# sideprotocol/plonky2-gpu

Measured on AMD Instinct MI355X. Metric: NTTs/sec at 2^20 Goldilocks, higher is better.
Workload: dtype u64 (Goldilocks, integer modular)

## Files before the change

plonky2_gpu_amd/csrc/capi.hip:

```cpp
#include <algorithm>
#include <list>
#include <map>
#include <mutex>
#include <string>
#include <vector>

#include <stdio.h>
#include <stdlib.h>
#include <string.h>

#include "../../include/plonky2_hip.h"
#include "gl_field.h"
#include "knobs.h"
#include "keccak.h"
#include "merkle.h"
#include "ntt.h"
#include "ntt_kernels.h"
#include "plonk.h"
#include "stark.h"
#include "fri.h"
#include "ed25519_gate_program.inc"

using namespace plonky2_hip;

// ... 1166 lines not shown

GlError gl_merkle_tree_from_columns_h(uint32_t hasher, const uint64_t *d_cols, uint32_t leaf_len, uint64_t n_leaves, uint64_t col_stride,
                                      uint32_t cap_height, uint64_t *d_digests, uint64_t *d_cap, void *ctx) {
    if (hasher == GL_HASHER_POSEIDON) return gl_merkle_tree_from_columns(d_cols, leaf_len, n_leaves, col_stride, cap_height, d_digests, d_cap, ctx);
    if (hasher != GL_HASHER_KECCAK25) return fail(GL_E_INVALID, "unknown hasher");
    DeviceCall device_call(ctx);
    if (!ctx || (!d_cols && leaf_len) || !d_cap) return fail(GL_E_INVALID, "null pointer");
    if (n_leaves == 0 || (n_leaves & (n_leaves - 1))) return fail(GL_E_INVALID, "n_leaves must be a power of two");
    if (cap_height > 63 || (1ull << cap_height) > n_leaves) return fail(GL_E_INVALID, "cap_height should be at most log2(leaves.len())");
    if ((1ull << cap_height) < n_leaves && !d_digests) return fail(GL_E_INVALID, "null pointer");
    if (leaf_len > 1 && col_stride < n_leaves) return fail(GL_E_INVALID, "col_stride smaller than n_leaves: the columns would overlap");
    if (leaf_len == 4) return fail(GL_E_INVALID, KECCAK_LEAF_LEN_4);
    HIP_TRY(keccak_merkle_tree(d_cols, 1, col_stride, leaf_len, n_leaves, cap_height, d_digests, d_cap, S(ctx)->stream));
    return ok();
}

GlError gl_merkle_tree_from_leaves_h(uint32_t hasher, const uint64_t *d_rows, uint32_t leaf_len, uint64_t n_leaves, uint32_t cap_height,
                                     uint64_t *d_digests, uint64_t *d_cap, void *ctx) {
    if (hasher == GL_HASHER_POSEIDON) return gl_merkle_tree_from_leaves(d_rows, leaf_len, n_leaves, cap_height, d_digests, d_cap, ctx);
    if (hasher != GL_HASHER_KECCAK25) return fail(GL_E_INVALID, "unknown hasher");
    DeviceCall device_call(ctx);
    if (!ctx || (!d_rows && leaf_len) || !d_cap) return fail(GL_E_INVALID, "null pointer");
    if (n_leaves == 0 || (n_leaves & (n_leaves - 1))) return fail(GL_E_INVALID, "n_leaves must be a power of two");
    if (cap_height > 63 || (1ull << cap_height) > n_leaves) return fail(GL_E_INVALID, "cap_height should be at most log2(leaves.len())");
    if ((1ull << cap_height) < n_leaves && !d_digests) return fail(GL_E_INVALID, "null pointer");
    if (leaf_len == 4) return fail(GL_E_INVALID, KECCAK_LEAF_LEN_4);
    HIP_TRY(keccak_merkle_tree(d_rows, leaf_len, 1, leaf_len, n_leaves, cap_height, d_digests, d_cap, S(ctx)->stream));
    return ok();
}

GlError gl_commit_from_coeffs_h(uint32_t hasher, const uint64_t *d_coeffs, uint64_t poly_num, uint32_t log_n, uint32_t rate_bits,
                                uint32_t cap_height, uint32_t salt_size, uint64_t shift, uint64_t *d_lde, uint64_t *d_leaves,
                                uint64_t *d_digests, uint64_t *d_cap, void *ctx) {
    if (hasher == GL_HASHER_POSEIDON)
        return gl_commit_from_coeffs(d_coeffs, poly_num, log_n, rate_bits, cap_height, salt_size, shift, d_lde, d_leaves, d_digests, d_cap, ctx);
    if (hasher != GL_HASHER_KECCAK25) return fail(GL_E_INVALID, "unknown hasher");
    DeviceCall device_call(ctx);
    return commit_from_coeffs_keccak(d_coeffs, poly_num, log_n, rate_bits, cap_height, salt_size, shift, d_lde, d_leaves, d_digests, d_cap, S(ctx));
}

GlError gl_commit_from_values_h(uint32_t hasher, uint64_t *d_values, uint64_t poly_num, uint32_t log_n, uint32_t rate_bits,
                                uint32_t cap_height, uint32_t salt_size, uint64_t shift, uint64_t *d_lde, uint64_t *d_leaves,
                                uint64_t *d_digests, uint64_t *d_cap, void *ctx) {
    if (hasher == GL_HASHER_POSEIDON)
        return gl_commit_from_values(d_values, poly_num, log_n, rate_bits, cap_height, salt_size, shift, d_lde, d_leaves, d_digests, d_cap, ctx);
    if (hasher != GL_HASHER_KECCAK25) return fail(GL_E_INVALID, "unknown hasher");
    DeviceCall device_call(ctx);
    if (const char *why = keccak_commit_argument_error(d_values, poly_num, log_n, rate_bits, cap_height, salt_size, d_lde, d_digests, d_cap, ctx))
        return fail(GL_E_INVALID, why);
    GlError e = gl_ntt_batch(d_values, poly_num, log_n, 1ull << log_n, 1, 0, ctx);
    if (e.code) return e;
    return gl_commit_from_coeffs_h(hasher, d_values, poly_num, log_n, rate_bits, cap_height, salt_size, shift, d_lde, d_leaves, d_digests, d_cap, ctx);
}

GlError gl_debug_copy(void *d_dst, const void *d_src, uint64_t bytes, void *ctx) {
    DeviceCall device_call(ctx);
    if (!ctx || !d_dst || !d_src) return fail(GL_E_INVALID, "null pointer");
    if ((bytes & 15) || (((uintptr_t)d_dst | (uintptr_t)d_src) & 15)) return fail(GL_E_INVALID, "16-byte granularity");
    if (bytes == 0) return ok();
    const uint64_t n16 = bytes / 16, per_block = 256ull * COPY_UNROLL;
    hipLaunchKernelGGL(copy16_kernel, dim3((unsigned)((n16 + per_block - 1) / per_block)), dim3(256), 0, S(ctx)->stream,
                       static_cast<const uint64_t *>(d_src), static_cast<uint64_t *>(d_dst), n16);
    HIP_TRY(hipGetLastError());
    return ok();
}

__global__ void radix_probe_kernel(int which, const uint64_t *in, uint64_t *out, uint64_t n_vec) {
    const uint64_t i = (uint64_t)blockIdx.x * blockDim.x + threadIdx.x;
    const uint64_t j = i < n_vec ? i : n_vec - 1;
    uint64_t v[16];
#pragma unroll
    for (int k = 0; k < 16; k++) v[k] = in[j * 16 + k];
    using namespace nttk;
    switch (which) {
        case 0: radix_dif_stage<4, 0, 0>(v); break;
        case 1: radix_dif_stage<4, 0, 1>(v); break;
        case 2: radix_dif_stage<4, 0, 2>(v); break;
        case 3: radix_dif_stage<4, 0, 3>(v); break;
        case 4: radix_dif<4, 0>(v); break;
        case 5: radix_dif_blocks<2>(v); break;
        case 6: shift_twiddles_radix4<0>(v); break;
        case 7: shift_twiddles_radix4<1>(v); break;
        case 8: shift_twiddles_radix4<2>(v); break;
        default: shift_twiddles_radix4<3>(v); break;
    }
    if (i < n_vec)
#pragma unroll
        for (int k = 0; k < 16; k++) out[i * 16 + k] = gl::canon(v[k]);
}

GlError gl_debug_field_op(int op, const uint64_t *d_a, const uint64_t *d_b, uint64_t *d_out, uint64_t n, void *ctx) {
    DeviceCall device_call(ctx);
    if (!ctx || !d_a || !d_out) return fail(GL_E_INVALID, "null pointer");
    if (n == 0) return ok();
    if (op >= 100 && op < 110) {
        if (n % 16) return fail(GL_E_INVALID, "ops 100-109 take vectors of sixteen elements");
        const uint64_t n_vec = n / 16;
        hipLaunchKernelGGL(radix_probe_kernel, dim3((unsigned)((n_vec + 255) / 256)), dim3(256), 0, S(ctx)->stream, op - 100, d_a, d_out, n_vec);
        HIP_TRY(hipGetLastError());
        return ok();
    }
    hipLaunchKernelGGL(field_op_kernel, dim3((unsigned)((n + 255) / 256)), dim3(256), 0, S(ctx)->stream, op, d_a, d_b,
                       d_out, n);
    HIP_TRY(hipGetLastError());
    return ok();
}


void init(void) {
    if (hipSetDevice(0) != hipSuccess) return;
    std::lock_guard<std::mutex> lk(g_mu);
    const NttTables *tb;
    (void)device_tables(0, &tb);
}

GlError ifft(uint64_t *d_values_flatten, int poly_num, int values_num_per_poly, int log_len,
             const uint64_t *d_root_table, const uint64_t *n_inv, void *ctx) {
    DeviceCall device_call(ctx);
    (void)d_root_table;
    if (poly_num < 0 || log_len < 0 || values_num_per_poly != (1 << log_len)) return fail(GL_E_INVALID, "bad sizes");
    if (n_inv) {
        uint64_t expect = glh::P - ((glh::P - 1) >> log_len);
        if (*n_inv % glh::P != expect) return fail(GL_E_INVALID, "n_inv does not equal 2^-log_len");
    }
    GlError e = gl_ntt_batch(d_values_flatten, (uint64_t)poly_num, (uint32_t)log_len, (uint64_t)values_num_per_poly, 1, 0, ctx);
    if (e.code) return e;
    HIP_TRY(hipStreamSynchronize(S(ctx)->stream));
    return ok();
}

GlError merkle_tree_from_coeffs(uint64_t *d_values_flatten, uint64_t *d_ext_values_flatten, int poly_num,
                                int values_num_per_poly, int log_len, const uint64_t *d_root_table,
                                const uint64_t *d_root_table2, const uint64_t *d_shift_powers, int rate_bits,
                                int salt_size, int cap_height, int pad_extvalues_len, void *ctx) {
    DeviceCall device_call(ctx);
    (void)d_root_table;
    (void)d_root_table2;
    (void)d_shift_powers;
    if (poly_num <= 0 || log_len < 0 || rate_bits < 0 || salt_size < 0 || cap_height < 0 || pad_extvalues_len < 0 ||
        values_num_per_poly != (1 << log_len))
        return fail(GL_E_INVALID, "bad sizes");
    if (log_len > 24) return fail(GL_E_INVALID, "log_len > 24 is not supported by this build");
    const uint64_t n_ext = (uint64_t)values_num_per_poly << rate_bits;
    const uint64_t ext_polys = (uint64_t)poly_num + salt_size;
    if ((uint64_t)pad_extvalues_len < ext_polys * n_ext)
        return fail(GL_E_INVALID, "pad_extvalues_len smaller than (poly_num+salt_size)*n_ext: regions would overlap");
    uint64_t *region_b = d_ext_values_flatten + pad_extvalues_len;
    uint64_t *digests = region_b + ext_polys * n_ext;
    uint64_t num_digests = 2 * (n_ext - (1ull << cap_height));
    GlError e = commit_from_coeffs_impl(d_values_flatten, (uint64_t)poly_num, (uint32_t)log_len, (uint32_t)rate_bits,
                                        (uint32_t)cap_height, (uint32_t)salt_size, 7, region_b, d_ext_values_flatten,
                                        digests, digests + 4 * num_digests, S(ctx), true);
    if (e.code) return e;
    HIP_TRY(hipStreamSynchronize(S(ctx)->stream));
    if (!PLONKY2_KNOB("PLONKY2_DROP_STREAM2_WAIT")) HIP_TRY(hipStreamSynchronize(S(ctx)->stream2));
    return ok();
}

GlError merkle_tree_from_values(uint64_t *d_values_flatten, uint64_t *d_ext_values_flatten, int poly_num,
                                int values_num_per_poly, int log_len, const uint64_t *d_root_table,
                                const uint64_t *d_root_table2, const uint64_t *d_shift_powers, const uint64_t *n_inv,
                                int rate_bits, int salt_size, int cap_height, int pad_extvalues_len, void *ctx) {
    DeviceCall device_call(ctx);
    GlError e = ifft(d_values_flatten, poly_num, values_num_per_poly, log_len, d_root_table, n_inv, ctx);
    if (e.code) return e;
    return merkle_tree_from_coeffs(d_values_flatten, d_ext_values_flatten, poly_num, values_num_per_poly, log_len,
                                   d_root_table, d_root_table2, d_shift_powers, rate_bits, salt_size, cap_height,
                                   pad_extvalues_len, ctx);
}

GlError build_merkle_tree(uint64_t *d_ext_values_flatten, int poly_num, int values_num_per_poly, int log_len,
                          int rate_bits, int salt_size, int cap_height, int pad_extvalues_len, void *ctx) {
    DeviceCall device_call(ctx);
    if (!ctx || !d_ext_values_flatten) return fail(GL_E_INVALID, "null pointer");
    if (poly_num <= 0 || log_len < 0 || rate_bits < 0 || salt_size < 0 || cap_height < 0 || pad_extvalues_len < 0 ||
        values_num_per_poly != (1 << log_len) || cap_height > log_len + rate_bits)
        return fail(GL_E_INVALID, "bad sizes");
    const uint32_t log_ext = (uint32_t)(log_len + rate_bits);
    const uint64_t n_ext = 1ull << log_ext, ext_polys = (uint64_t)poly_num + salt_size;
// ... 169 lines not shown
```

plonky2_gpu_amd/csrc/ntt_direct.hip:

```cpp

#include "ntt_kernels.h"

namespace plonky2_hip {
namespace nttk {

namespace {

#ifndef NTT_TAIL_GROUPED
#define NTT_TAIL_GROUPED 1
#endif
#ifndef DIRECT_DIAG_HOOKS
#define DIRECT_TILE_BARRIER() lds_barrier()
#define DIRECT_LOAD_TILE(t) (t)
#define DIRECT_STORE_TILE(t) (t)
#define DIRECT_DIAG_TAIL_FRONT_ON 0
#define DIRECT_DIAG_SAME_STORES_ON 0
#define DIRECT_NT_LOAD_COL false
#define DIRECT_NT_STORE_COL false
#define DIRECT_NT_LOAD_ROW false
#define DIRECT_NT_STORE_ROW false
#define DIRECT_TOUCH_STATE
#define DIRECT_TOUCH_COL(t_in_a)
#define DIRECT_TOUCH_ROW(t_in_a)
#endif

__device__ __forceinline__ uint64_t lds_ld(const unsigned char *lds, uint32_t off) { return *reinterpret_cast<const uint64_t *>(lds + off); }
__device__ __forceinline__ void lds_st(unsigned char *lds, uint32_t off, uint64_t v) { *reinterpret_cast<uint64_t *>(lds + off) = v; }
template <bool NT = false>
__device__ __forceinline__ uint64_t g_ld(const uint64_t *base, uint32_t byte_off) {
    const uint64_t *q = reinterpret_cast<const uint64_t *>(reinterpret_cast<const unsigned char *>(base) + byte_off);
    if constexpr (NT) return __builtin_nontemporal_load(q);
    return *q;
}
template <bool NT = false>
__device__ __forceinline__ void g_st(uint64_t *base, uint32_t byte_off, uint64_t v) {
    uint64_t *q = reinterpret_cast<uint64_t *>(reinterpret_cast<unsigned char *>(base) + byte_off);
    if constexpr (NT)
        __builtin_nontemporal_store(v, q);
    else
        *q = v;
}
constexpr bool NT_LOAD_COL = DIRECT_NT_LOAD_COL, NT_STORE_COL = DIRECT_NT_STORE_COL, NT_LOAD_ROW = DIRECT_NT_LOAD_ROW, NT_STORE_ROW = DIRECT_NT_STORE_ROW;

template <int LOGG>
struct ColGeom {
    static constexpr int G = 1 << LOGG, LOGC = 6 - LOGG, C = 1 << LOGC, LOGR = 8 + LOGG, R = 1 << LOGR;
    static constexpr uint32_t ROWB = C * 8;
    static constexpr uint32_t SA = 16 * ROWB + (G >= 4 ? ROWB : 0);
    static constexpr uint32_t XBYTES = 16 * G * SA;
    static constexpr uint32_t TWBYTES = 16 * G * 16 * 8;
    static constexpr uint32_t LDS_BYTES = XBYTES + TWBYTES;
    static constexpr uint32_t cu_entries(uint32_t gz) { return gz * (G > 1 ? G * 16 : 256); }
    static constexpr uint32_t t2z_entries(uint32_t gz) { return G > 1 ? gz * 16 * G : 0; }
    static constexpr uint32_t cs_entries(uint32_t gz) { return gz * C; }
    static constexpr uint32_t coset_bytes(uint32_t gz) { return (cu_entries(gz) + t2z_entries(gz) + cs_entries(gz)) * 8; }
};

static_assert(ColGeom<3>::LDS_BYTES <= 160 * 1024 && ColGeom<2>::LDS_BYTES <= 160 * 1024, "the exchange image and the tables must fit the 160 KiB of LDS of a gfx950 CU");

template <int LOGG, bool NATURAL, bool COSET = false, bool FINAL = false, bool REVIN = false>
__global__ __launch_bounds__(1024) __attribute__((amdgpu_waves_per_eu(4, 4))) void ntt_col_direct_kernel(const PassParams p, const uint32_t gx, const uint32_t gy, const uint32_t gz, const uint32_t per_b) {
    using GEO = ColGeom<LOGG>;
    constexpr int G = GEO::G, LOGC = GEO::LOGC, C = GEO::C, LOGR = GEO::LOGR;
    constexpr uint32_t ROWB = GEO::ROWB, SA = GEO::SA;
    extern __shared__ __attribute__((aligned(16))) unsigned char ldsb[];
    unsigned char *X = ldsb;
    unsigned char *TW = ldsb + GEO::XBYTES;
    unsigned char *CU = TW + GEO::TWBYTES, *T2Z = CU + GEO::cu_entries(gz) * 8, *CS = T2Z + GEO::t2z_entries(gz) * 8;

    const uint32_t tid = threadIdx.x, lane = tid & 63;
    const uint32_t wave = __builtin_amdgcn_readfirstlane(tid >> 6);
    const uint32_t g = lane >> LOGC, c = lane & (C - 1);

    const uint32_t W = gridDim.x;
    const uint32_t u = (W & 7) == 0 ? (blockIdx.x & 7) * (W >> 3) + (blockIdx.x >> 3) : blockIdx.x;
    const uint32_t P = gy * gz;
    uint32_t b0, bstep, p0, pstep;
    if (per_b) {
        if constexpr (COSET) b0 = u / per_b, p0 = u % per_b;
        else b0 = u % gx, p0 = u / gx;
        bstep = gx, pstep = per_b;
    } else {
        b0 = u, bstep = W, p0 = 0, pstep = 1;
    }
    const uint32_t np_local = p0 < P ? (P - p0 + pstep - 1) / pstep : 0;
    const uint32_t nb_local = b0 < gx ? (gx - b0 + bstep - 1) / bstep : 0;
    const uint32_t n_tiles = np_local * nb_local;
    if (n_tiles == 0) return;

    for (uint32_t e = tid; e < 16u * G * 16u; e += 1024) {
        const uint32_t w_ = e / (16 * G), g_ = (e / 16) % G, ka = e % 16;
        reinterpret_cast<uint64_t *>(TW)[e] = p.twh[(ka * (16 * g_ + w_)) << (12 - LOGR)];
    }
    uint64_t t2[G > 1 ? G : 1];
    if constexpr (!COSET)
        static_for<1, G>([&](auto K_) {
            constexpr int kb = decltype(K_)::value;
            t2[kb] = p.twh[(kb * wave) << (12 - 4 - LOGG)];
        });
    if constexpr (COSET) {
        auto cs_pow = [&](uint32_t z, uint64_t ex) { return gl::mul(p.cs_hi[z * p.cs_hi_len + (uint32_t)(ex >> 10)], p.cs_lo[z * 1024 + (uint32_t)(ex & 1023)]); };
        for (uint32_t e = tid; e < GEO::cu_entries(gz); e += 1024) {
            const uint32_t i = e & 15, mid = G > 1 ? 16 * ((e >> 4) % G) : (e >> 4) & 15, z = G > 1 ? e / (16 * G) : e >> 8;
            reinterpret_cast<uint64_t *>(CU)[e] = cs_pow(z, (uint64_t)p.in_m * (((uint32_t)i << (LOGR - 4)) + mid));
        }
        for (uint32_t e = tid; e < GEO::t2z_entries(gz); e += 1024) {
            const uint32_t kb = e % G, w_ = (e / G) & 15, z = e / (16 * G);
            reinterpret_cast<uint64_t *>(T2Z)[e] = gl::mul(p.twh[(kb * w_) << (12 - 4 - LOGG)], cs_pow(z, (uint64_t)p.in_m * w_));
        }
        for (uint32_t e = tid; e < GEO::cs_entries(gz); e += 1024)
            reinterpret_cast<uint64_t *>(CS)[e] = cs_pow(e / C, (uint64_t)b0 * C + (e % C));
    }

    const uint32_t tw_base = (wave * G + g) * 128;
    const uint32_t lane_x = wave * ROWB + c * 8;
    const uint32_t pw_base = 16 * g * SA + lane_x;
    const uint32_t pr_base = g * SA + lane_x;
    constexpr bool natural = NATURAL;
    auto opaque_lane = [&]() {
        uint32_t l = lane;
        asm volatile("" : "+v"(l));
        return l;
    };
    auto kab_of = [&](uint32_t l) { return G * wave + (l >> LOGC); };
    auto xr_base_of = [&](uint32_t l) { return kab_of(l) * SA + (l & (C - 1)) * 8; };
    auto ld_off_of = [&](uint32_t l) { return (uint32_t)(((l & (C - 1)) + (uint64_t)(16 * (l >> LOGC) + wave) * p.in_m) * 8); };
    const uint64_t out_c = p.out_c ? p.out_c : 1;
    auto st_off_of = [&](uint32_t l) {
        const uint32_t kab = kab_of(l);
        const uint32_t out_row_lane = natural ? kab : (brev_rt(kab & 15, 4) << (LOGR - 4)) | (brev_rt(kab >> 4, LOGG) << 4);
        return (uint32_t)(((l & (C - 1)) * out_c + (uint64_t)out_row_lane * p.out_m) * 8);
    };

    auto tile_of = [&](uint32_t t, uint32_t &b, uint32_t &a, uint32_t &z) {
        const uint32_t bi = t / np_local, pi = t - bi * np_local;
        b = b0 + bi * bstep;
        const uint32_t pp = p0 + pi * pstep;
        if constexpr (COSET) a = pp / gz, z = pp % gz;
        else a = pp % gy, z = pp / gy;
        if (p.sweep_down) a = gy - 1 - a;
    };

    uint64_t A[16];
    const uint32_t ld_step = (uint32_t)(((uint64_t)p.in_m << (LOGR - 4)) * 8);
    auto issue_loads = [&](uint32_t t) {
        uint32_t b, a, z;
        tile_of(DIRECT_LOAD_TILE(t), b, a, z);
        if constexpr (REVIN) {
            static_assert(!COSET && NATURAL, "the reversed-input pass is the first pass of a natural-order inverse transform");
            const uint64_t *base = p.src + (a * p.in_sa + z * p.in_sz);
            const uint32_t l = opaque_lane();
            const uint32_t L = b * C + (l & (C - 1)), m0 = 16 * (l >> LOGC) + wave;
            const uint32_t cols = (uint32_t)p.in_m;
            uint32_t off = L ? (((uint32_t)GEO::R - 1 - m0) * cols + (cols - L)) * 8 : (((uint32_t)GEO::R - m0) * cols) * 8;
            const bool wraps = L == 0 && m0 == 0;
            static_for<0, 16>([&](auto I_) {
                constexpr int i = decltype(I_)::value;
                if constexpr (i == 0) A[i] = g_ld<NT_LOAD_COL>(base, wraps ? 0u : off);
                else A[i] = g_ld<NT_LOAD_COL>(base, off);
                if constexpr (i < 15) off -= ld_step;
            });
            return;
        }
        const uint64_t *base = p.src + (a * p.in_sa + b * p.in_sb + z * p.in_sz);
        uint32_t off = ld_off_of(opaque_lane());
        static_for<0, 16>([&](auto I_) {
            constexpr int i = decltype(I_)::value;
            A[i] = g_ld<NT_LOAD_COL>(base, off);
            if constexpr (i < 15) off += ld_step;
        });
    };

    uint64_t B[16];
    uint64_t cc0 = 1, cstep = 1;
    constexpr bool kept_twiddles = !COSET && !FINAL;
    uint64_t cw[kept_twiddles ? 8 : 1], cstep8 = 1;
    uint32_t chain_b = 0xFFFFFFFFu;
    const uint32_t st_row = (uint32_t)(p.out_m * 8);

    uint64_t cc = 1;
    uint64_t *obase = p.dst;
    uint32_t so = 0;
    auto tail_begin = [&](uint32_t k) {
        uint32_t b, a, z;
        tile_of(k, b, a, z);
        if (!FINAL && b != chain_b) {
            chain_b = b;
            const uint32_t l = opaque_lane();
            const uint64_t L = (uint64_t)b * C + (l & (C - 1));
            cc0 = wpow(p, L * kab_of(l));
            if (p.chain_scale != 1) cc0 = gl::mul(cc0, p.chain_scale);
            cstep = wpow(p, L << (4 + LOGG));
            asm volatile("" : "+v"(cc0), "+v"(cstep));
            if constexpr (kept_twiddles) {
                cw[0] = cc0;
                static_for<1, 8>([&](auto J_) {
                    constexpr int j = decltype(J_)::value;
                    cw[j] = gl::mul(cw[j - 1], cstep);
                });
                const uint64_t s2 = gl::mul(cstep, cstep), s4 = gl::mul(s2, s2);
                cstep8 = gl::mul(s4, s4);
            }
        }
        if constexpr (DIRECT_DIAG_SAME_STORES_ON) tile_of(0, b, a, z);
        obase = p.dst + (a * p.out_sa + b * p.out_sb + (COSET ? brev_rt(z, p.rate_bits) : z) * p.out_sz);
        if constexpr (COSET) cc = gl::mul(cc0, lds_ld(CS, (z * C + (opaque_lane() & (C - 1))) * 8));
        else cc = cc0;
        so = st_off_of(opaque_lane());
    };
    auto tail_unit = [&](auto J_) {
        constexpr int j = decltype(J_)::value;
        constexpr int s3 = brev_c(j, 4);
        if constexpr (FINAL) {
            B[s3] = gl::canon(B[s3]);
        } else if constexpr (kept_twiddles) {
            if constexpr (j < 8) B[s3] = gl::mul(B[s3], cw[j]);
            else B[s3] = gl::mul(B[s3], gl::mul(cw[j - 8], cstep8));
        } else {
            B[s3] = gl::mul(B[s3], cc);
            if constexpr (j < 15) cc = gl::mul(cc, cstep);
        }
        const uint32_t row = natural ? (uint32_t)(j << (4 + LOGG)) : (uint32_t)s3;
        g_st<NT_STORE_COL>(obase, so + row * st_row, B[s3]);
        __builtin_amdgcn_sched_barrier(0);
    };
    auto tail_store = [&](auto J_) {
        constexpr int j = decltype(J_)::value;
        constexpr int s3 = brev_c(j, 4);
        const uint32_t row = natural ? (uint32_t)(j << (4 + LOGG)) : (uint32_t)s3;
        g_st<NT_STORE_COL>(obase, so + row * st_row, B[s3]);
        __builtin_amdgcn_sched_barrier(0);
    };
    auto tail_units = [&](auto LO_, auto HI_) {
        constexpr int LO = decltype(LO_)::value, HI = decltype(HI_)::value, N = HI - LO;
        if constexpr (NTT_TAIL_GROUPED && kept_twiddles && N >= 1 && N <= 8) {
            uint64_t tw[N];
            constexpr int N_HI = HI > 8 ? HI - (LO > 8 ? LO : 8) : 0;
            if constexpr (N_HI > 0)
                rare_group<N_HI>([&](auto I_, gl::rare_mask &f) { constexpr int j = (LO > 8 ? LO : 8) + decltype(I_)::value; tw[j - LO] = gl::mul_f(cw[j - 8], cstep8, f); },
                                 [&](auto I_, gl::rare_mask f) { constexpr int j = (LO > 8 ? LO : 8) + decltype(I_)::value; tw[j - LO] = gl::mul_fix(tw[j - LO], f); });
            rare_group<N>(
                [&](auto I_, gl::rare_mask &f) {
                    constexpr int j = LO + decltype(I_)::value, s3 = brev_c(j, 4);
                    if constexpr (j < 8) B[s3] = gl::mul_f(B[s3], cw[j], f);
                    else B[s3] = gl::mul_f(B[s3], tw[j - LO], f);
                },
                [&](auto I_, gl::rare_mask f) {
                    constexpr int s3 = brev_c(LO + decltype(I_)::value, 4);
                    B[s3] = gl::mul_fix(B[s3], f);
                });
            static_for<LO, HI>([&](auto J_) { tail_store(J_); });
        } else {
            static_for<LO, HI>([&](auto J_) { tail_unit(J_); });
        }
    };

    DIRECT_TOUCH_STATE
    auto first_rounds = [&](auto WITH_TAIL_, uint32_t t_in_a) {
        constexpr bool with_tail = decltype(WITH_TAIL_)::value;
        uint32_t zc = 0;
        if constexpr (COSET) {
            uint32_t b_, a_;
            tile_of(t_in_a, b_, a_, zc);
        }
        if constexpr (with_tail && DIRECT_DIAG_TAIL_FRONT_ON) tail_units(std::integral_constant<int, 0>{}, std::integral_constant<int, 16>{});
#define TAIL(lo, hi) do { if constexpr (with_tail && !DIRECT_DIAG_TAIL_FRONT_ON) tail_units(std::integral_constant<int, lo>{}, std::integral_constant<int, hi>{}); } while (0)
        TAIL(0, 4);
        if constexpr (COSET) {
            const uint32_t cu_base = (G > 1 ? (zc * G + (opaque_lane() >> LOGC)) * 16 : (zc * 16 + wave) * 16) * 8;
            mul_run<0, 16>(A, [](auto I_) { return decltype(I_)::value; }, [&](auto I_) { return lds_ld(CU, cu_base + decltype(I_)::value * 8); }, [](auto) {});
        }
        radix_dif_stage<4, 0, 3>(A);
        DIRECT_TOUCH_COL(t_in_a);
        TAIL(4, 6);
        radix_dif_stage<4, 0, 2>(A);
        TAIL(6, 8);
        radix_dif_stage<4, 0, 1>(A);
        TAIL(8, 10);
        radix_dif_stage<4, 0, 0>(A);
        TAIL(10, 12);
        mul_run<1, 16>(A, [](auto S_) { return decltype(S_)::value; }, [&](auto S_) { return lds_ld(TW, tw_base + brev_c(decltype(S_)::value, 4) * 8); },
                       [&](auto S_) {
                           constexpr int s = decltype(S_)::value;
                           if constexpr (s == 5) TAIL(12, 13);
                           if constexpr (s == 10) TAIL(13, 14);
                       });
        if constexpr (G > 1) {
            static_for<0, 16>([&](auto S_) {
                constexpr int s = decltype(S_)::value;
                constexpr int ka = brev_c(s, 4);
                lds_st(X, pw_base + ka * SA, A[s]);
            });
            tile_sync<64>();
            static_for<0, 16 / G>([&](auto J_) {
                constexpr int j = decltype(J_)::value;
                static_for<0, G>([&](auto GG_) {
                    constexpr int gg = decltype(GG_)::value;
                    A[j * G + gg] = lds_ld(X, pr_base + (16 * gg + G * j) * SA);
                });
            });
            tile_sync<64>();
            radix_dif_blocks<LOGG>(A);
            TAIL(14, 15);
            if constexpr (COSET)
                mul_run<0, 16>(A, [](auto E_) { return decltype(E_)::value; },
                               [&](auto E_) { return lds_ld(T2Z, ((zc * 16 + wave) * G + brev_c(decltype(E_)::value % G, LOGG)) * 8); }, [](auto) {});
            else
                mul_run<0, (G - 1) * (16 / G)>(A, [](auto K_) { return (decltype(K_)::value / (G - 1)) * G + 1 + decltype(K_)::value % (G - 1); },
                                               [&](auto K_) { return t2[brev_c(1 + decltype(K_)::value % (G - 1), LOGG)]; }, [](auto) {});
            static_for<0, 16 / G>([&](auto J_) {
                constexpr int j = decltype(J_)::value;
                static_for<0, G>([&](auto S_) {
                    constexpr int s2 = decltype(S_)::value;
                    constexpr int kb = brev_c(s2, LOGG);
                    lds_st(X, pr_base + (G * j + 16 * kb) * SA, A[j * G + s2]);
                });
            });
            TAIL(15, 16);
        } else {
            TAIL(14, 16);
            static_for<0, 16>([&](auto S_) {
                constexpr int s = decltype(S_)::value;
                constexpr int ka = brev_c(s, 4);
                lds_st(X, pr_base + ka * SA, A[s]);
            });
        }
#undef TAIL
    };

    lds_barrier();
    issue_loads(0);
    const uint32_t last = n_tiles - 1;
    first_rounds(std::false_type{}, 0);
    if (last > 0) issue_loads(1);
#pragma unroll 1
    for (uint32_t k = 0; k <= last; k++) {
        DIRECT_TILE_BARRIER();
        const uint32_t xr_base = xr_base_of(opaque_lane());
        static_for<0, 16>([&](auto WR_) {
            constexpr int wr = decltype(WR_)::value;
            B[wr] = lds_ld(X, xr_base + wr * ROWB);
        });
        DIRECT_TILE_BARRIER();
        radix_dif<4, 0>(B);
        tail_begin(k);
        if (k < last) {
            first_rounds(std::true_type{}, k + 1);
            if (k + 1 < last) issue_loads(k + 2);
        } else {
            tail_units(std::integral_constant<int, 0>{}, std::integral_constant<int, 16>{});
        }
    }
}

template <int LOGG, bool NATURAL, bool COSET = false, bool FINAL = false, bool REVIN = false>
hipError_t launch_col_direct_t(const PassParams &p, dim3 grid, hipStream_t stream) {
    using GEO = ColGeom<LOGG>;
    const uint32_t lds_bytes = GEO::LDS_BYTES + (COSET ? GEO::coset_bytes(grid.z) : 0);
    static DynamicLds attr;
    if (hipError_t e = allow_dynamic_lds(attr, reinterpret_cast<const void *>(&ntt_col_direct_kernel<LOGG, NATURAL, COSET, FINAL, REVIN>), lds_bytes); e != hipSuccess) return e;
    int dev = 0, cus = 256;
    if (hipGetDevice(&dev) == hipSuccess) (void)hipDeviceGetAttribute(&cus, hipDeviceAttributeMultiprocessorCount, dev);
    const uint64_t pairs = (uint64_t)grid.y * grid.z, total = pairs * grid.x;
    if (total == 0) return hipSuccess;
    if (total > 0xFFFFFFFFull) return hipErrorInvalidValue;
    uint32_t per_b = 0, wgs;
    if (grid.x <= (uint32_t)cus) {
        per_b = (uint32_t)cus / grid.x;
        if (per_b > pairs) per_b = (uint32_t)pairs;
        wgs = grid.x * per_b;
    } else {
        wgs = (uint32_t)cus;
    }
    if (COSET && per_b == 0) return hipErrorInvalidValue;
    hipLaunchKernelGGL((ntt_col_direct_kernel<LOGG, NATURAL, COSET, FINAL, REVIN>), dim3(wgs), dim3(1024), lds_bytes, stream, p, (uint32_t)grid.x, (uint32_t)grid.y, (uint32_t)grid.z, per_b);
    return hipGetLastError();
}


struct RowGeom {
    static constexpr uint32_t SQ = 136, SB = 544, SA = 8736;
    static constexpr uint32_t XBYTES = 16 * SA;
    static constexpr uint32_t TW1_STRIDE = 136, TW1_BYTES = 64 * TW1_STRIDE;
    static constexpr uint32_t TW2_STRIDE = 136, TW2_BYTES = 4 * TW2_STRIDE;
    static constexpr uint32_t LDS_BYTES = XBYTES + TW1_BYTES;
};

template <bool INVERSE>
__global__ __launch_bounds__(1024) __attribute__((amdgpu_waves_per_eu(4, 4))) void ntt_row_natural_direct_kernel(const PassParams p, const uint32_t gx, const uint32_t gy, const uint32_t gz) {
    using GEO = RowGeom;
    constexpr uint32_t SQ = GEO::SQ, SB = GEO::SB, SA = GEO::SA;
    extern __shared__ __attribute__((aligned(16))) unsigned char ldsb[];
    unsigned char *X = ldsb;
    unsigned char *TW1 = ldsb + GEO::XBYTES;

    const uint32_t tid = threadIdx.x, lane = tid & 63;
    const uint32_t wave = __builtin_amdgcn_readfirstlane(tid >> 6);

    const uint32_t W = gridDim.x;
    const uint32_t u = (W & 7) == 0 ? (blockIdx.x & 7) * (W >> 3) + (blockIdx.x >> 3) : blockIdx.x;
    const uint32_t total = gx * gy * gz;
    if (u >= total) return;
    const uint32_t n_tiles = (total - u + W - 1) / W;

    for (uint32_t e = tid; e < 64 * 16; e += 1024) {
        const uint32_t l = e >> 4, ka = e & 15;
        *reinterpret_cast<uint64_t *>(TW1 + l * GEO::TW1_STRIDE + ka * 8) = p.twh[(ka * l) << 2];
    }

    const uint32_t q = lane & 3, hi4 = lane >> 2;
    const uint32_t tw1_base = lane * GEO::TW1_STRIDE;
    const uint32_t pw_base = hi4 * SB + q * SQ + wave * 8;
    const uint32_t pr_base = hi4 * SA + q * SQ + wave * 8;
    auto opaque_lane = [&]() {
        uint32_t l = lane;
        asm volatile("" : "+v"(l));
        return l;
    };

    auto tile_of = [&](uint32_t t, uint32_t &b, uint32_t &a, uint32_t &z) {
        const uint32_t id = u + t * W;
        b = id % gx;
        const uint32_t r = id / gx;
        a = r % gy;
        z = r / gy;
        if (p.sweep_down) a = gy - 1 - a;
    };

    uint64_t A[16];
    auto issue_loads = [&](uint32_t t) {
        uint32_t b, a, z;
        tile_of(DIRECT_LOAD_TILE(t), b, a, z);
        const uint32_t row = (b * 16 + wave + p.row_shift) & (p.t_limit - 1);
        const uint64_t *base = p.src + (a * p.in_sa + z * p.in_sz + (uint64_t)row * p.in_t);
// ... 360 lines not shown
```

plonky2_gpu_amd/csrc/ntt_kernels.h:

```cpp
#pragma once
#include <atomic>
#include <hip/hip_runtime.h>
#include <stdint.h>

#include <type_traits>

#include "gl_field.h"

namespace plonky2_hip {
namespace nttk {

enum : uint32_t { F_LOAD_ROWS = 1, F_STORE_ROWS = 2, F_NATURAL = 4, F_INVERSE = 8, F_COSET = 16,
                  F_WIDE = 32,
                  F_RAW_OUT = 64,
                  F_FINAL_COL = 128 };

struct PassParams {
    const uint64_t *src;
    uint64_t *dst;
    const uint64_t *twl;
    const uint64_t *twh;
    const uint64_t *cs_hi;
    const uint64_t *cs_lo;
    uint64_t in_sa, in_sb, in_sz, in_t, in_m;
// ... 105 lines not shown
    static_assert(NB % GB == 0, "whole groups");
    static_for<0, NB / GB>([&](auto G_) {
        constexpr int g0 = decltype(G_)::value * GB;
        gl::rare_mask fa[GB], fs[GB];
        static_for<0, GB>([&](auto B_) {
            constexpr int b = g0 + decltype(B_)::value, k = decltype(B_)::value, bb = b % NBP;
            constexpr int i0 = BASE + (b / NBP) * (1 << D) + (bb / half) * 2 * half + (bb % half), i1 = i0 + half;
            constexpr int K = (39 * (bb % half) * (32 >> s)) % 192;
            gl::bfly_f<(K >= 96)>(v[i0], v[i1], v[i0], v[i1], fa[k], fs[k]);
        });
        __builtin_amdgcn_sched_barrier(RARE_FENCE_MASK);
        gl::rare_mask any = 0;
        static_for<0, GB>([&](auto B_) { any |= fa[decltype(B_)::value] | fs[decltype(B_)::value]; });
        if (GL_RARE_ANY(any)) {
            static_for<0, GB>([&](auto B_) {
                constexpr int b = g0 + decltype(B_)::value, k = decltype(B_)::value, bb = b % NBP;
                constexpr int i0 = BASE + (b / NBP) * (1 << D) + (bb / half) * 2 * half + (bb % half), i1 = i0 + half;
                v[i0] = gl::add_fix(v[i0], fa[k]);
                v[i1] = gl::sub_fix(v[i1], fs[k]);
            });
        }
    });
    if constexpr (s > 0) {
        static_assert(NB <= 8, "the shift twiddles of a stage form one group");
        gl::rare_mask fm[NB];
        static_for<0, NB>([&](auto B_) {
            constexpr int b = decltype(B_)::value, bb = b % NBP;
            constexpr int i1 = BASE + (b / NBP) * (1 << D) + (bb / half) * 2 * half + (bb % half) + half;
            constexpr int K = (39 * (bb % half) * (32 >> s)) % 192, KK = K >= 96 ? K - 96 : K;
            v[i1] = gl::mul_pow2_f<KK>(v[i1], fm[b]);
        });
        __builtin_amdgcn_sched_barrier(RARE_FENCE_MASK);
        gl::rare_mask any = 0;
        static_for<0, NB>([&](auto B_) { any |= fm[decltype(B_)::value]; });
        if (GL_RARE_ANY(any)) {
            static_for<0, NB>([&](auto B_) {
                constexpr int b = decltype(B_)::value, bb = b % NBP;
                constexpr int i1 = BASE + (b / NBP) * (1 << D) + (bb / half) * 2 * half + (bb % half) + half;
                constexpr int K = (39 * (bb % half) * (32 >> s)) % 192, KK = K >= 96 ? K - 96 : K;
                v[i1] = gl::mul_pow2_fix<KK>(v[i1], fm[b]);
            });
        }
    }
}

template <int N, class One, class Fix>
__device__ __forceinline__ void rare_group(One &&one, Fix &&fix) {
    static_assert(N >= 1 && N <= 8, "a group's masks must fit the scalar registers a kernel has to spare");
    gl::rare_mask f[N];
    static_for<0, N>([&](auto I_) { one(I_, f[decltype(I_)::value]); });
    __builtin_amdgcn_sched_barrier(RARE_FENCE_MASK);
    gl::rare_mask any = 0;
    static_for<0, N>([&](auto I_) { any |= f[decltype(I_)::value]; });
    if (GL_RARE_ANY(any)) static_for<0, N>([&](auto I_) { fix(I_, f[decltype(I_)::value]); });
}

template <int LO, int HI, class Idx, class W, class After>
__device__ __forceinline__ void mul_run(uint64_t (&v)[16], Idx &&idx, W &&w, After &&after) {
    constexpr int N = HI - LO;
    static_for<0, (N + 7) / 8>([&](auto G_) {
        constexpr int k0 = LO + 8 * decltype(G_)::value, n = (HI - k0) < 8 ? (HI - k0) : 8;
        rare_group<n>(
            [&](auto I_, gl::rare_mask &f) {
                constexpr int k = k0 + decltype(I_)::value;
                auto K_ = std::integral_constant<int, k>{};
                v[idx(K_)] = gl::mul_f(v[idx(K_)], w(K_), f);
                after(K_);
            },
            [&](auto I_, gl::rare_mask f) {
                constexpr int k = k0 + decltype(I_)::value;
                auto K_ = std::integral_constant<int, k>{};
                v[idx(K_)] = gl::mul_fix(v[idx(K_)], f);
            });
    });
}

template <int D, int BASE>
__device__ __forceinline__ void radix_dif(uint64_t (&v)[16]) {
    static_for<0, D>([&](auto S_) { radix_dif_stage<D, BASE, D - 1 - decltype(S_)::value>(v); });
}
template <int D>
__device__ __forceinline__ void radix_dif_blocks(uint64_t (&v)[16]) {
    static_for<0, D>([&](auto S_) { radix_dif_stage<D, 0, D - 1 - decltype(S_)::value, (16 >> D)>(v); });
}

template <int KBHI>
__device__ __forceinline__ void shift_twiddles_radix4(uint64_t (&v)[16]) {
    constexpr auto KQ = [](int kblo, int q) { return (39 * q * (4 * KBHI + kblo)) % 192; };
    constexpr auto NEGQ = [](int kblo, int q) { return (39 * q * (4 * KBHI + kblo)) % 192 >= 96; };
    {
        gl::rare_mask fm[12];
        static_for<0, 12>([&](auto I_) {
            constexpr int i = decltype(I_)::value, kblo = i / 3, q = 1 + i % 3, KK = KQ(kblo, q) % 96;
            v[4 * kblo + q] = gl::mul_pow2_f<KK>(v[4 * kblo + q], fm[i]);
        });
        __builtin_amdgcn_sched_barrier(RARE_FENCE_MASK);
        gl::rare_mask any = 0;
        static_for<0, 12>([&](auto I_) { any |= fm[decltype(I_)::value]; });
        if (GL_RARE_ANY(any))
            static_for<0, 12>([&](auto I_) {
                constexpr int i = decltype(I_)::value, kblo = i / 3, q = 1 + i % 3, KK = KQ(kblo, q) % 96;
                v[4 * kblo + q] = gl::mul_pow2_fix<KK>(v[4 * kblo + q], fm[i]);
            });
    }
    auto bfly = [&](auto CNEG_, auto I0_, auto I1_, gl::rare_mask &f0, gl::rare_mask &f1) {
        constexpr bool cneg = decltype(CNEG_)::value;
        constexpr int i0 = decltype(I0_)::value, i1 = decltype(I1_)::value;
        if constexpr (cneg) gl::bfly_f<false>(v[i0], v[i1], v[i1], v[i0], f1, f0);
        else gl::bfly_f<false>(v[i0], v[i1], v[i0], v[i1], f0, f1);
    };
    auto fix = [&](auto IS_SUM_, auto SHIFT_, auto I_, gl::rare_mask f, gl::rare_mask fshift) {
        constexpr bool is_sum = decltype(IS_SUM_)::value;
        constexpr int shift = decltype(SHIFT_)::value, i = decltype(I_)::value;
        if constexpr (shift == 0) {
            v[i] = is_sum ? gl::add_fix(v[i], f) : gl::sub_fix(v[i], f);
        } else {
            v[i] = gl::mul_pow2_fix<shift>(v[i], fshift);
            const uint64_t c = gl::masked_const<gl::eps_times_pow2(shift)>(f);
            v[i] = is_sum ? gl::add(v[i], c) : gl::sub(v[i], c);
        }
    };
    using std::integral_constant;
    using std::bool_constant;
    {
        gl::rare_mask f0[8], f1[8], fm[4];
        static_for<0, 4>([&](auto B_) {
            constexpr int kblo = decltype(B_)::value, b = 4 * kblo;
            bfly(bool_constant<NEGQ(kblo, 2)>{}, integral_constant<int, b>{}, integral_constant<int, b + 2>{}, f0[2 * kblo], f1[2 * kblo]);
            bfly(bool_constant<NEGQ(kblo, 1) != NEGQ(kblo, 3)>{}, integral_constant<int, b + 1>{}, integral_constant<int, b + 3>{}, f0[2 * kblo + 1], f1[2 * kblo + 1]);
        });
        static_for<0, 4>([&](auto B_) {
            constexpr int kblo = decltype(B_)::value;
            v[4 * kblo + 3] = gl::mul_pow2_f<48>(v[4 * kblo + 3], fm[kblo]);
        });
        __builtin_amdgcn_sched_barrier(RARE_FENCE_MASK);
        gl::rare_mask any = 0;
        static_for<0, 8>([&](auto I_) { any |= f0[decltype(I_)::value] | f1[decltype(I_)::value]; });
        static_for<0, 4>([&](auto I_) { any |= fm[decltype(I_)::value]; });
        if (GL_RARE_ANY(any))
            static_for<0, 4>([&](auto B_) {
                constexpr int kblo = decltype(B_)::value, b = 4 * kblo;
                constexpr bool na = NEGQ(kblo, 2), nb = NEGQ(kblo, 1) != NEGQ(kblo, 3);
                fix(bool_constant<!na>{}, integral_constant<int, 0>{}, integral_constant<int, b>{}, f0[2 * kblo], 0);
                fix(bool_constant<na>{}, integral_constant<int, 0>{}, integral_constant<int, b + 2>{}, f1[2 * kblo], 0);
                fix(bool_constant<!nb>{}, integral_constant<int, 0>{}, integral_constant<int, b + 1>{}, f0[2 * kblo + 1], 0);
                fix(bool_constant<nb>{}, integral_constant<int, 48>{}, integral_constant<int, b + 3>{}, f1[2 * kblo + 1], fm[kblo]);
            });
    }
    {
        gl::rare_mask f0[8], f1[8];
        static_for<0, 4>([&](auto B_) {
            constexpr int kblo = decltype(B_)::value, b = 4 * kblo;
            bfly(bool_constant<NEGQ(kblo, 1)>{}, integral_constant<int, b>{}, integral_constant<int, b + 1>{}, f0[2 * kblo], f1[2 * kblo]);
            bfly(bool_constant<NEGQ(kblo, 1)>{}, integral_constant<int, b + 2>{}, integral_constant<int, b + 3>{}, f0[2 * kblo + 1], f1[2 * kblo + 1]);
        });
        __builtin_amdgcn_sched_barrier(RARE_FENCE_MASK);
        gl::rare_mask any = 0;
        static_for<0, 8>([&](auto I_) { any |= f0[decltype(I_)::value] | f1[decltype(I_)::value]; });
        if (GL_RARE_ANY(any))
            static_for<0, 4>([&](auto B_) {
                constexpr int kblo = decltype(B_)::value, b = 4 * kblo;
                constexpr bool n1 = NEGQ(kblo, 1);
                fix(bool_constant<!n1>{}, integral_constant<int, 0>{}, integral_constant<int, b>{}, f0[2 * kblo], 0);
                fix(bool_constant<n1>{}, integral_constant<int, 0>{}, integral_constant<int, b + 1>{}, f1[2 * kblo], 0);
                fix(bool_constant<!n1>{}, integral_constant<int, 0>{}, integral_constant<int, b + 2>{}, f0[2 * kblo + 1], 0);
                fix(bool_constant<n1>{}, integral_constant<int, 0>{}, integral_constant<int, b + 3>{}, f1[2 * kblo + 1], 0);
// ... 50 lines not shown
```

Measured before the change: 132,500.

## Fold per-wave t2 twiddles into shifted radix-16 DIF via power-of-two multiplies

For non-coset column passes with G of 2 or 4, the per-wave inter-group twiddle multiplies (t2, loaded from the twiddle table and applied with full Goldilocks multiplies) are removed. They are absorbed into a specialised radix-16 DIF whose butterflies multiply by constant powers of two, since these twiddles are 64th roots of unity and so are powers of 2 mod p. The tile loop is wrapped in a lambda instantiated per wave class, which increases code size. Lane-base computation is moved inside that lambda, with opaque registers for the divisors to steer register allocation. Probe ops are added to test the new butterfly.

```diff
diff --git a/plonky2_gpu_amd/csrc/capi.hip b/plonky2_gpu_amd/csrc/capi.hip
--- a/plonky2_gpu_amd/csrc/capi.hip
+++ b/plonky2_gpu_amd/csrc/capi.hip
@@ -1272,7 +1272,11 @@
         case 6: shift_twiddles_radix4<0>(v); break;
         case 7: shift_twiddles_radix4<1>(v); break;
         case 8: shift_twiddles_radix4<2>(v); break;
-        default: shift_twiddles_radix4<3>(v); break;
+        case 9: shift_twiddles_radix4<3>(v); break;
+        case 10: radix16_dif_shifted<0>(v); break;
+        case 11: radix16_dif_shifted<1>(v); break;
+        case 12: radix16_dif_shifted<2>(v); break;
+        default: radix16_dif_shifted<3>(v); break;
     }
     if (i < n_vec)
 #pragma unroll
@@ -1283,8 +1287,8 @@
     DeviceCall device_call(ctx);
     if (!ctx || !d_a || !d_out) return fail(GL_E_INVALID, "null pointer");
     if (n == 0) return ok();
-    if (op >= 100 && op < 110) {
-        if (n % 16) return fail(GL_E_INVALID, "ops 100-109 take vectors of sixteen elements");
+    if (op >= 100 && op < 114) {
+        if (n % 16) return fail(GL_E_INVALID, "ops 100-113 take vectors of sixteen elements");
         const uint64_t n_vec = n / 16;
         hipLaunchKernelGGL(radix_probe_kernel, dim3((unsigned)((n_vec + 255) / 256)), dim3(256), 0, S(ctx)->stream, op - 100, d_a, d_out, n_vec);
         HIP_TRY(hipGetLastError());
diff --git a/plonky2_gpu_amd/csrc/ntt_direct.hip b/plonky2_gpu_amd/csrc/ntt_direct.hip
--- a/plonky2_gpu_amd/csrc/ntt_direct.hip
+++ b/plonky2_gpu_amd/csrc/ntt_direct.hip
@@ -70,7 +70,6 @@
 
     const uint32_t tid = threadIdx.x, lane = tid & 63;
     const uint32_t wave = __builtin_amdgcn_readfirstlane(tid >> 6);
-    const uint32_t g = lane >> LOGC, c = lane & (C - 1);
 
     const uint32_t W = gridDim.x;
     const uint32_t u = (W & 7) == 0 ? (blockIdx.x & 7) * (W >> 3) + (blockIdx.x >> 3) : blockIdx.x;
@@ -92,14 +91,15 @@
         const uint32_t w_ = e / (16 * G), g_ = (e / 16) % G, ka = e % 16;
         reinterpret_cast<uint64_t *>(TW)[e] = p.twh[(ka * (16 * g_ + w_)) << (12 - LOGR)];
     }
+    constexpr bool t2_as_shifts = !COSET && (G == 2 || G == 4);
     uint64_t t2[G > 1 ? G : 1];
-    if constexpr (!COSET)
+    if constexpr (!COSET && !t2_as_shifts)
         static_for<1, G>([&](auto K_) {
             constexpr int kb = decltype(K_)::value;
             t2[kb] = p.twh[(kb * wave) << (12 - 4 - LOGG)];
         });
     if constexpr (COSET) {
-        auto cs_pow = [&](uint32_t z, uint64_t ex) { return gl::mul(p.cs_hi[z * p.cs_hi_len + (uint32_t)(ex >> 10)], p.cs_lo[z * 1024 + (uint32_t)(ex & 1023)]); };
+        auto cs_pow = [&](uint32_t z, uint64_t ex) __attribute__((always_inline)) { return gl::mul(p.cs_hi[z * p.cs_hi_len + (uint32_t)(ex >> 10)], p.cs_lo[z * 1024 + (uint32_t)(ex & 1023)]); };
         for (uint32_t e = tid; e < GEO::cu_entries(gz); e += 1024) {
             const uint32_t i = e & 15, mid = G > 1 ? 16 * ((e >> 4) % G) : (e >> 4) & 15, z = G > 1 ? e / (16 * G) : e >> 8;
             reinterpret_cast<uint64_t *>(CU)[e] = cs_pow(z, (uint64_t)p.in_m * (((uint32_t)i << (LOGR - 4)) + mid));
@@ -112,38 +112,46 @@
             reinterpret_cast<uint64_t *>(CS)[e] = cs_pow(e / C, (uint64_t)b0 * C + (e % C));
     }
 
-    const uint32_t tw_base = (wave * G + g) * 128;
-    const uint32_t lane_x = wave * ROWB + c * 8;
-    const uint32_t pw_base = 16 * g * SA + lane_x;
-    const uint32_t pr_base = g * SA + lane_x;
     constexpr bool natural = NATURAL;
-    auto opaque_lane = [&]() {
-        uint32_t l = lane;
+    uint32_t lane_v = lane;
+    uint32_t np_div = np_local, gy_div = gy;
+    auto opaque_lane = [&]() __attribute__((always_inline)) {
+        uint32_t l = lane_v;
         asm volatile("" : "+v"(l));
         return l;
     };
-    auto kab_of = [&](uint32_t l) { return G * wave + (l >> LOGC); };
-    auto xr_base_of = [&](uint32_t l) { return kab_of(l) * SA + (l & (C - 1)) * 8; };
-    auto ld_off_of = [&](uint32_t l) { return (uint32_t)(((l & (C - 1)) + (uint64_t)(16 * (l >> LOGC) + wave) * p.in_m) * 8); };
+    uint32_t tw_base, pw_base, pr_base;
+    auto lane_bases = [&]() __attribute__((always_inline)) {
+        lane_v = __builtin_amdgcn_mbcnt_hi(~0u, __builtin_amdgcn_mbcnt_lo(~0u, 0u));
+        asm volatile("" : "+s"(np_div), "+s"(gy_div));
+        const uint32_t l = opaque_lane(), g = l >> LOGC, c = l & (C - 1);
+        const uint32_t lane_x = wave * ROWB + c * 8;
+        tw_base = (wave * G + g) * 128;
+        pw_base = 16 * g * SA + lane_x;
+        pr_base = g * SA + lane_x;
+    };
+    auto kab_of = [&](uint32_t l) __attribute__((always_inline)) { return G * wave + (l >> LOGC); };
+    auto xr_base_of = [&](uint32_t l) __attribute__((always_inline)) { return kab_of(l) * SA + (l & (C - 1)) * 8; };
+    auto ld_off_of = [&](uint32_t l) __attribute__((always_inline)) { return (uint32_t)(((l & (C - 1)) + (uint64_t)(16 * (l >> LOGC) + wave) * p.in_m) * 8); };
     const uint64_t out_c = p.out_c ? p.out_c : 1;
-    auto st_off_of = [&](uint32_t l) {
+    auto st_off_of = [&](uint32_t l) __attribute__((always_inline)) {
         const uint32_t kab = kab_of(l);
         const uint32_t out_row_lane = natural ? kab : (brev_rt(kab & 15, 4) << (LOGR - 4)) | (brev_rt(kab >> 4, LOGG) << 4);
         return (uint32_t)(((l & (C - 1)) * out_c + (uint64_t)out_row_lane * p.out_m) * 8);
     };
 
-    auto tile_of = [&](uint32_t t, uint32_t &b, uint32_t &a, uint32_t &z) {
-        const uint32_t bi = t / np_local, pi = t - bi * np_local;
+    auto tile_of = [&](uint32_t t, uint32_t &b, uint32_t &a, uint32_t &z) __attribute__((always_inline)) {
+        const uint32_t bi = t / np_div, pi = t - bi * np_div;
         b = b0 + bi * bstep;
         const uint32_t pp = p0 + pi * pstep;
         if constexpr (COSET) a = pp / gz, z = pp % gz;
-        else a = pp % gy, z = pp / gy;
+        else a = pp % gy_div, z = pp / gy_div;
         if (p.sweep_down) a = gy - 1 - a;
     };
 
     uint64_t A[16];
     const uint32_t ld_step = (uint32_t)(((uint64_t)p.in_m << (LOGR - 4)) * 8);
-    auto issue_loads = [&](uint32_t t) {
+    auto issue_loads = [&](uint32_t t) __attribute__((always_inline)) {
         uint32_t b, a, z;
         tile_of(DIRECT_LOAD_TILE(t), b, a, z);
         if constexpr (REVIN) {
@@ -181,7 +189,7 @@
     uint64_t cc = 1;
     uint64_t *obase = p.dst;
     uint32_t so = 0;
-    auto tail_begin = [&](uint32_t k) {
+    auto tail_begin = [&](uint32_t k) __attribute__((always_inline)) {
         uint32_t b, a, z;
         tile_of(k, b, a, z);
         if (!FINAL && b != chain_b) {
@@ -208,7 +216,7 @@
         else cc = cc0;
         so = st_off_of(opaque_lane());
     };
-    auto tail_unit = [&](auto J_) {
+    auto tail_unit = [&](auto J_) __attribute__((always_inline)) {
         constexpr int j = decltype(J_)::value;
         constexpr int s3 = brev_c(j, 4);
         if constexpr (FINAL) {
@@ -224,14 +232,14 @@
         g_st<NT_STORE_COL>(obase, so + row * st_row, B[s3]);
         __builtin_amdgcn_sched_barrier(0);
     };
-    auto tail_store = [&](auto J_) {
+    auto tail_store = [&](auto J_) __attribute__((always_inline)) {
         constexpr int j = decltype(J_)::value;
         constexpr int s3 = brev_c(j, 4);
         const uint32_t row = natural ? (uint32_t)(j << (4 + LOGG)) : (uint32_t)s3;
         g_st<NT_STORE_COL>(obase, so + row * st_row, B[s3]);
         __builtin_amdgcn_sched_barrier(0);
     };
-    auto tail_units = [&](auto LO_, auto HI_) {
+    auto tail_units = [&](auto LO_, auto HI_) __attribute__((always_inline)) {
         constexpr int LO = decltype(LO_)::value, HI = decltype(HI_)::value, N = HI - LO;
         if constexpr (NTT_TAIL_GROUPED && kept_twiddles && N >= 1 && N <= 8) {
             uint64_t tw[N];
@@ -256,7 +264,7 @@
     };
 
     DIRECT_TOUCH_STATE
-    auto first_rounds = [&](auto WITH_TAIL_, uint32_t t_in_a) {
+    auto first_rounds = [&](auto WITH_TAIL_, uint32_t t_in_a) __attribute__((always_inline)) {
         constexpr bool with_tail = decltype(WITH_TAIL_)::value;
         uint32_t zc = 0;
         if constexpr (COSET) {
@@ -305,7 +313,7 @@
             if constexpr (COSET)
                 mul_run<0, 16>(A, [](auto E_) { return decltype(E_)::value; },
                                [&](auto E_) { return lds_ld(T2Z, ((zc * 16 + wave) * G + brev_c(decltype(E_)::value % G, LOGG)) * 8); }, [](auto) {});
-            else
+            else if constexpr (!t2_as_shifts)
                 mul_run<0, (G - 1) * (16 / G)>(A, [](auto K_) { return (decltype(K_)::value / (G - 1)) * G + 1 + decltype(K_)::value % (G - 1); },
                                                [&](auto K_) { return t2[brev_c(1 + decltype(K_)::value % (G - 1), LOGG)]; }, [](auto) {});
             static_for<0, 16 / G>([&](auto J_) {
@@ -328,28 +336,42 @@
 #undef TAIL
     };
 
+    const uint32_t last = n_tiles - 1;
+    auto run_tiles = [&](auto E0_) __attribute__((always_inline)) {
+        constexpr int E0 = decltype(E0_)::value;
+        lane_bases();
+        issue_loads(0);
+        first_rounds(std::false_type{}, 0);
+        if (last > 0) issue_loads(1);
+#pragma unroll 1
+        for (uint32_t k = 0; k <= last; k++) {
+            DIRECT_TILE_BARRIER();
+            const uint32_t xr_base = xr_base_of(opaque_lane());
+            static_for<0, 16>([&](auto WR_) {
+                constexpr int wr = decltype(WR_)::value;
+                B[wr] = lds_ld(X, xr_base + wr * ROWB);
+            });
+            DIRECT_TILE_BARRIER();
+            if constexpr (E0 == 0) radix_dif<4, 0>(B);
+            else radix16_dif_shifted<E0>(B);
+            tail_begin(k);
+            if (k < last) {
+                first_rounds(std::true_type{}, k + 1);
+                if (k + 1 < last) issue_loads(k + 2);
+            } else {
+                tail_units(std::integral_constant<int, 0>{}, std::integral_constant<int, 16>{});
+            }
+        }
+    };
     lds_barrier();
-    issue_loads(0);
-    const uint32_t last = n_tiles - 1;
-    first_rounds(std::false_type{}, 0);
-    if (last > 0) issue_loads(1);
-#pragma unroll 1
-    for (uint32_t k = 0; k <= last; k++) {
-        DIRECT_TILE_BARRIER();
-        const uint32_t xr_base = xr_base_of(opaque_lane());
-        static_for<0, 16>([&](auto WR_) {
-            constexpr int wr = decltype(WR_)::value;
-            B[wr] = lds_ld(X, xr_base + wr * ROWB);
-        });
-        DIRECT_TILE_BARRIER();
-        radix_dif<4, 0>(B);
-        tail_begin(k);
-        if (k < last) {
-            first_rounds(std::true_type{}, k + 1);
-            if (k + 1 < last) issue_loads(k + 2);
-        } else {
-            tail_units(std::integral_constant<int, 0>{}, std::integral_constant<int, 16>{});
-        }
+    if constexpr (t2_as_shifts) {
+        const uint32_t kb = wave >> (4 - LOGG);
+        if (kb == 0) run_tiles(std::integral_constant<int, 0>{});
+        else if (G == 2 || kb == 2) run_tiles(std::integral_constant<int, 2>{});
+        else if (kb == 1) run_tiles(std::integral_constant<int, 1>{});
+        else run_tiles(std::integral_constant<int, 3>{});
+    } else {
+        run_tiles(std::integral_constant<int, 0>{});
     }
 }
 
diff --git a/plonky2_gpu_amd/csrc/ntt_kernels.h b/plonky2_gpu_amd/csrc/ntt_kernels.h
--- a/plonky2_gpu_amd/csrc/ntt_kernels.h
+++ b/plonky2_gpu_amd/csrc/ntt_kernels.h
@@ -211,6 +211,64 @@
 template <int D>
 __device__ __forceinline__ void radix_dif_blocks(uint64_t (&v)[16]) {
     static_for<0, D>([&](auto S_) { radix_dif_stage<D, 0, D - 1 - decltype(S_)::value, (16 >> D)>(v); });
+}
+
+constexpr unsigned char DIF_SHIFT_EXP[4][4][8] = {
+    {{  0,  48, 120, 168, 156,  12,  84, 132}, {  0,  48, 120, 168,   0,   0,   0,   0}, {  0,  48,   0,   0,   0,   0,   0,   0}, {  0,   0,   0,   0,   0,   0,   0,   0}},
+    {{ 39,  87, 159,  15,   3,  51, 123, 171}, { 78, 126,   6,  54,   0,   0,   0,   0}, {156,  12,   0,   0,   0,   0,   0,   0}, {120,   0,   0,   0,   0,   0,   0,   0}},
+    {{ 78, 126,   6,  54,  42,  90, 162,  18}, {156,  12,  84, 132,   0,   0,   0,   0}, {120, 168,   0,   0,   0,   0,   0,   0}, { 48,   0,   0,   0,   0,   0,   0,   0}},
+    {{117, 165,  45,  93,  81, 129,   9,  57}, { 42,  90, 162,  18,   0,   0,   0,   0}, { 84, 132,   0,   0,   0,   0,   0,   0}, {168,   0,   0,   0,   0,   0,   0,   0}},
+};
+constexpr int dif_shift_block_offset(int s, int blk) {
+    int e = 0;
+    for (int d = 0; d < 3 - s; d++) e += ((blk >> (3 - s - 1 - d)) & 1) * (4 << d);
+    return e;
+}
+constexpr bool dif_shift_table_ok() {
+    for (int e0 = 0; e0 < 4; e0++)
+        for (int s = 0; s < 4; s++)
+            for (int blk = 0; blk < (8 >> s); blk++)
+                if (DIF_SHIFT_EXP[e0][s][blk] != (39 * ((e0 + dif_shift_block_offset(s, blk)) << s)) % 192) return false;
+    return true;
+}
+static_assert(dif_shift_table_ok(), "T = w_64^(E N / 2) = 2^(39 E N / 2)");
+constexpr int dif_shift_exponent(int e0, int s, int blk) { return DIF_SHIFT_EXP[e0][s][blk]; }
+
+template <int E0, int s>
+__device__ __forceinline__ void radix16_dif_shifted_stage(uint64_t (&v)[16]) {
+    constexpr int half = 1 << s;
+    gl::rare_mask fm[8], f0[8], f1[8];
+    static_for<0, 8>([&](auto B_) {
+        constexpr int b = decltype(B_)::value, blk = b / half, i1 = blk * 2 * half + (b % half) + half;
+        constexpr int KK = dif_shift_exponent(E0, s, blk) % 96;
+        if constexpr (KK != 0) v[i1] = gl::mul_pow2_f<KK>(v[i1], fm[b]);
+        else fm[b] = 0;
+    });
+    static_for<0, 8>([&](auto B_) {
+        constexpr int b = decltype(B_)::value, blk = b / half, i0 = blk * 2 * half + (b % half), i1 = i0 + half;
+        if constexpr (dif_shift_exponent(E0, s, blk) >= 96) gl::bfly_f<false>(v[i0], v[i1], v[i1], v[i0], f1[b], f0[b]);
+        else gl::bfly_f<false>(v[i0], v[i1], v[i0], v[i1], f0[b], f1[b]);
+    });
+    __builtin_amdgcn_sched_barrier(RARE_FENCE_MASK);
+    gl::rare_mask any = 0;
+    static_for<0, 8>([&](auto B_) { constexpr int b = decltype(B_)::value; any |= fm[b] | f0[b] | f1[b]; });
+    if (GL_RARE_ANY(any)) {
+        static_for<0, 8>([&](auto B_) {
+            constexpr int b = decltype(B_)::value, blk = b / half, i0 = blk * 2 * half + (b % half), i1 = i0 + half;
+            constexpr int K = dif_shift_exponent(E0, s, blk), KK = K % 96;
+            constexpr int isum = K >= 96 ? i1 : i0, idif = K >= 96 ? i0 : i1;
+            v[isum] = gl::add_fix(v[isum], K >= 96 ? f1[b] : f0[b]);
+            v[idif] = gl::sub_fix(v[idif], K >= 96 ? f0[b] : f1[b]);
+            if constexpr (KK % 32 != 0 && KK >= 32) {
+                v[isum] = gl::sub(v[isum], gl::masked_const<gl::eps_times_pow2(0)>(fm[b]));
+                v[idif] = gl::add(v[idif], gl::masked_const<gl::eps_times_pow2(0)>(fm[b]));
+            }
+        });
+    }
+}
+template <int E0>
+__device__ __forceinline__ void radix16_dif_shifted(uint64_t (&v)[16]) {
+    static_for<0, 4>([&](auto S_) { radix16_dif_shifted_stage<E0, 3 - decltype(S_)::value>(v); });
 }
 
 template <int KBHI>
```

Result: slower. 130,900 (-1.2%).
